# helloybz/CLANE

Measured on AMD Instinct MI355X. Metric: embedding-update iters/sec (Jacobi sweeps of Z <- X + gamma*P*Z, P frozen), higher is better.
Workload: dtype f32; 1 GPU; R-MAT |V|=2000000 |E|=40000000 d=256 f32, gamma=0.76, CosineSimilarity (reference mode), seeds 3/4

## Files before the change

### clane_amd/_hip.py

```python
from __future__ import annotations

import abc
import ctypes as C
import os
import threading
from pathlib import Path
from typing import Optional

import torch

LIB_NAME = "libclane_hip.so"
LIB_PATH = Path(__file__).resolve().parent / LIB_NAME
ABI_VERSION = 5

SCORE_REFERENCE, SCORE_PER_EDGE, SCORE_RAW_DOT = 0, 1, 2
SPMM_SINKS_UNTOUCHED = 1
SPMM_TABLE_BEYOND_CACHE = 2
SCORE_FUSE_SOFTMAX = 1
SCORE_MODES = {"reference": SCORE_REFERENCE, "per_edge": SCORE_PER_EDGE, "raw_dot": SCORE_RAW_DOT}

_p, _i64, _i32 = C.c_void_p, C.c_int64, C.c_int32

SIGNATURES = {
    "clane_abi_version": (C.c_int, []),
# ... 29 lines not shown
    SIGNATURES[f"clane_spmm_update_class_{_s}"] = (
        C.c_int,
        [_p, _p, _p, _p, _p, _i64, _i32, _p, _p, _i64, _i64, _p, _i64, _p, _i64, _g, _p, _i64, _i32, _i32, _p, _p, _p, _p])
    SIGNATURES[f"clane_edge_score_class_{_s}"] = (
        C.c_int, [_p, _p, _p, _p, _p, _p, _i64, _i32, _p, _p, _i64, _i64, _p, _i64, _i32, _i32, _p, _p, _p, _i32, _p, _p])
    SIGNATURES[f"clane_gather_rows_{_s}"] = (C.c_int, [_p, _i64, _p, _i64, _i32, _p, _i64, _p])
    SIGNATURES[f"clane_l1_distance_{_s}"] = (C.c_int, [_p, _i64, _p, _i64, _i64, _i32, _p, _p, _p, _p])
for _s in ("f32", "f64"):
    SIGNATURES[f"clane_degree_weighted_sums_{_s}"] = (C.c_int, [_p, _p, _p, _i64, _p, _p, _p])
    SIGNATURES[f"clane_edge_score_finalize_{_s}"] = (C.c_int, [_p, _p, _i64, _i64, _i32, _p, _p, _p, _p])
    SIGNATURES[f"clane_segment_softmax_{_s}"] = (C.c_int, [_p, _i64, _p, _i64, _i64, _p, _i64, _p])
    SIGNATURES[f"clane_pair_cosine_{_s}"] = (C.c_int, [_p, _i64, _p, _i64, _i64, _i32, _p, _p, _p])
    SIGNATURES[f"clane_edge_score_pair_{_s}"] = (
        C.c_int, [_p, _p, _i64, _i64, _p, _i64, _p, _i64, _i32, _p, _i32, _i64, _p, _i64, _p])
    SIGNATURES[f"clane_edge_score_class_pair_{_s}"] = (
        C.c_int, [_p, _p, _p, _p, _p, _p, _i64, _i32, _p, _p, _i64, _i64, _p, _i64, _p, _i64, _i32, _p, _i32, _p, _p])
for _s in ("f32", "f64", "bf16"):
    SIGNATURES[f"clane_project_rows_{_s}"] = (C.c_int, [_p, _i64, _i32, _i64, _p, _p, _i64, _p])
    SIGNATURES[f"clane_pair_project_{_s}"] = (C.c_int, [_p, _i64, _i32, _i64, _p, _p, _i64, _p, _p, _p, _p])
    SIGNATURES[f"clane_pair_grad_{_s}"] = (C.c_int, [_p, _i64, _i32, _i64, _p, _p, _i64, _p, _p, _p, _p, _p, _p, _p])
for _s in ("f32", "f64"):
    SIGNATURES[f"clane_pair_loss_{_s}"] = (C.c_int, [_p, _p, _i64, _i32, _p, _p, _p, _p, _p, _p, _p])
    SIGNATURES[f"clane_adam_step_{_s}"] = (C.c_int, [_p, _p, _p, _p, _i64, C.c_double, _p, _p, _p])
SIGNATURES["clane_pair_grad_ws_len"] = (_i64, [_i64, _i32])
SIGNATURES["clane_pair_labels"] = (C.c_int, [_p, _p, _i64, _p, _p, _i64, _p, _p])

_SUFFIX = {torch.float32: "f32", torch.float64: "f64", torch.bfloat16: "bf16"}
_ACC = {torch.float32: torch.float32, torch.float64: torch.float64, torch.bfloat16: torch.float32}
VEC_ELEMS = {torch.float32: 4, torch.float64: 2, torch.bfloat16: 8}


class ClaneHipError(RuntimeError):
    pass


class _MirrorStruct(C.Structure):
    _fields_ = [("row_ptr", _p), ("slot", _p), ("bufs", _p), ("ld", _i64), ("aligned16", _i32)]


MIRROR_ROW_BITS = 28


class Mirror:

    def __init__(self, row_ptr: torch.Tensor, slot: torch.Tensor, bufs):
        if row_ptr.dtype != torch.int64 or slot.dtype != torch.int32 or not (row_ptr.is_contiguous()
# ... 204 lines not shown
    def edge_score_class_pair(self, rowptr, colidx, item_e0, item_len, item_slot, item_row, items_per_block,
                              class_rows, slot_ptr, row0, S, N, d, scores, stats=None, fuse_softmax=False,
                              n_slots=None, row_parts=1):
        raise NotImplementedError(f"{type(self).__name__} has no edge_score_class_pair")

    def pair_project(self, Z, d: int, src, dst, W, A, Bm):
        raise NotImplementedError(f"{type(self).__name__} has no pair_project")

    def pair_loss(self, A, Bm, d: int, linked, u, g, mask, ws, stats):
        raise NotImplementedError(f"{type(self).__name__} has no pair_loss")

    def pair_grad_ws_len(self, B: int, d: int) -> int:
        raise NotImplementedError(f"{type(self).__name__} has no pair_grad_ws_len")

    def pair_grad(self, Z, d: int, src, dst, A, Bm, g, stats, ws, dW):
        raise NotImplementedError(f"{type(self).__name__} has no pair_grad")

    def adam_step(self, W, m, v, dW, lr: float, stats, state):
        raise NotImplementedError(f"{type(self).__name__} has no adam_step")

    def pair_labels(self, rowptr, colidx, nrows: int, src, dst, linked):
        raise NotImplementedError(f"{type(self).__name__} has no pair_labels")

    def bind(self, method: str, *args, **kwargs):
        fn = getattr(self, method)
        return lambda: fn(*args, **kwargs)


class HipKernels(KernelBackend):

    def __init__(self, lib: Optional[C.CDLL] = None):
        self.lib = lib if lib is not None else load_library()
        self._tls = threading.local()

    def _invoke(self, fn, what: str, *cargs):
        rec = getattr(self._tls, "recording", None)
        if rec is not None:
            rec.append((fn, cargs, what))
        else:
            self._check(fn(*cargs), what)

    def bind(self, method: str, *args, **kwargs):
        self._tls.recording = []
        try:
            getattr(self, method)(*args, **kwargs)
            (fn, cargs, what), = self._tls.recording
        finally:
            self._tls.recording = None
        check = self._check
        return lambda: check(fn(*cargs), what)

    def _check(self, rc: int, what: str):
# ... 136 lines not shown
                     _mirror_arg(mirror, Z_new.dtype), _vec(partials, torch.float64, "partials"), self._stream(Z_old))

    def spmm_split_slab_len(self, n_segments: int, d: int) -> int:
        return int(self.lib.clane_spmm_split_slab_len(n_segments, d))

    def spmm_update_split(self, rowptr, colidx, P, split_rows, seg_ptr, seg_row, edges_per_segment: int, row0: int,
                          Z_old, X, gamma: float, Z_new, d: int, slab, partials, mirror: Optional[Mirror] = None):
        zo, ldz = _mat(Z_old, "Z_old")
        xp, ldx = _mat(X, "X")
        zn, ldo = _mat(Z_new, "Z_new")
        self._invoke(self._fn("clane_spmm_update_split", Z_old.dtype), "clane_spmm_update_split",
                     _vec(rowptr, torch.int64, "rowptr"), _vec(colidx, torch.int32, "colidx"),
                     _vec(P, acc_dtype(Z_old.dtype), "P"), _vec(split_rows, torch.int32, "split_rows"),
                     _vec(seg_ptr, torch.int64, "seg_ptr"), _vec(seg_row, torch.int32, "seg_row"),
                     split_rows.numel(), seg_row.numel(), edges_per_segment, row0, zo, ldz, xp, ldx, gamma, zn, ldo, d,
                     _vec(slab, acc_dtype(Z_old.dtype), "slab"), _mirror_arg(mirror, Z_new.dtype),
                     _vec(partials, torch.float64, "partials"), self._stream(Z_old))

    def spmm_class_slab_len(self, n_slots: int, d: int) -> int:
        return int(self.lib.clane_spmm_class_slab_len(n_slots, d))

    def spmm_update_class(self, colidx, P, item_e0, item_len, item_slot, items_per_block: int, class_rows, slot_ptr,
                          row0: int, Z_old, X, gamma: float, Z_new, d: int, slab, partials,
                          mirror: Optional[Mirror] = None, beyond_cache: bool = False):
        zo, ldz = _mat(Z_old, "Z_old")
        xp, ldx = _mat(X, "X")
        zn, ldo = _mat(Z_new, "Z_new")
        n_items = item_e0.numel()
        if n_items % items_per_block or item_len.numel() != n_items or item_slot.numel() != n_items:
            raise ValueError("spmm_update_class: the item arrays must hold whole blocks of items_per_block items")
        self._invoke(self._fn("clane_spmm_update_class", Z_old.dtype), "clane_spmm_update_class",
                     _vec(colidx, torch.int32, "colidx"), _vec(P, acc_dtype(Z_old.dtype), "P"),
                     _vec(item_e0, torch.int64, "item_e0"), _vec(item_len, torch.int32, "item_len"),
                     _vec(item_slot, torch.int32, "item_slot"), n_items // items_per_block, items_per_block,
                     _vec(class_rows, torch.int32, "class_rows"), _vec(slot_ptr, torch.int64, "slot_ptr"),
                     class_rows.numel(), row0, zo, ldz, xp, ldx, gamma, zn, ldo, d,
                     SPMM_TABLE_BEYOND_CACHE if beyond_cache else 0,
                     _vec(slab, acc_dtype(Z_old.dtype), "slab"), _mirror_arg(mirror, Z_new.dtype),
                     _vec(partials, torch.float64, "partials"), self._stream(Z_old))

    def reduce_partials(self, partials, n: int, ws, out):
        self._invoke(self.lib.clane_reduce_partials, "clane_reduce_partials",
                     _vec(partials, torch.float64, "partials"), n, _vec(ws, torch.float64, "ws"),
                     _vec(out, torch.float64, "out"), self._stream(out))

    def l1_distance(self, A, B, d: int, ws, out, sq_a: Optional[torch.Tensor] = None):
        ap, lda = _mat(A, "A")
        bp, ldb = _mat(B, "B")
        self._check(self._fn("clane_l1_distance", A.dtype)(
            ap, lda, bp, ldb, A.shape[0], d, self._sq_arg(sq_a, A.dtype), _vec(ws, torch.float64, "ws"),
            _vec(out, torch.float64, "out"), self._stream(A)), "clane_l1_distance")

    def gather_rows(self, src, idx, d: int, dst):
# ... 144 lines not shown
```

### clane_amd/csrc/clane_abi.hip

```cpp
#include "../../include/clane_hip.h"

#include <hip/hip_runtime.h>

#include <climits>
#include <cstdarg>
#include <cstdio>
#include <cstring>

#include "build_p.h"
#include "edge_score.h"
#include "device_utils.h"
#include "pair_train.h"
#include "projection.h"
#include "spmm_update.h"

namespace {

using namespace clane;

thread_local char g_err[512] = "";

int fail(int code, const char *fmt, ...) {
    va_list ap;
    va_start(ap, fmt);
// ... 446 lines not shown
    const Layout L = pick_layout<T>(d, {Z_old, X, Z_new, mirror_alignment_probe(mirror, Z_new)},
                                    {ldz, ldx, ldo, mirror && mirror->row_ptr ? mirror->ld : ldo});
    const int64_t ld_slab = ceil_div(d, 8) * 8;
    const Mirror<T> mir = make_mirror<T>(mirror);
    dispatch_layout<T>(L, [&]<int VEC, int LPR>() {
        constexpr int U = VEC > 1 ? CLANE_LONG_U : 4;
        constexpr int kDeepU = (LPR == 32 && VEC == 4 && sizeof(T) == 4) ? CLANE_CLASS_U32
                               : (LPR == 16 && VEC == 8 && sizeof(T) == 2) ? CLANE_CLASS_U16B : 0;
        if (n_blocks > 0 && kDeepU > 0 && (flags & CLANE_SPMM_TABLE_BEYOND_CACHE))
            spmm_class_chunk_kernel<T, PT, VEC, LPR, (kDeepU > 0 ? kDeepU : U)>
                <<<unsigned(n_blocks), kBlock, 0, (hipStream_t)stream>>>(
                    colidx, P, item_e0, item_len, item_slot, items_per_block, Z_old, ldz, d, slab, ld_slab);
        else if (n_blocks > 0)
            spmm_class_chunk_kernel<T, PT, VEC, LPR, U><<<unsigned(n_blocks), kBlock, 0, (hipStream_t)stream>>>(
                colidx, P, item_e0, item_len, item_slot, items_per_block, Z_old, ldz, d, slab, ld_slab);
        spmm_class_combine_kernel<T, VEC, LPR>
            <<<unsigned(ceil_div(n_rows, kWave / LPR)), kCombineWaves * kWave, 0, (hipStream_t)stream>>>(
            class_rows, slot_ptr, n_rows, row0, slab, ld_slab, Z_old, ldz, X, ldx, gamma, Z_new, ldo, d, mir,
            (flags & CLANE_SPMM_TABLE_BEYOND_CACHE) != 0, delta_partials);
    });
    return check_launch("spmm_update_class");
}

template <typename T>
int l1_distance(const T *A, int64_t lda, const T *B, int64_t ldb, int64_t nrows, int32_t d,
                typename Elem<T>::acc_t *sq_a, double *ws, double *out, void *stream) {
    REQUIRE(nrows >= 0 && d > 0 && lda >= d && ldb >= d, "l1_distance: bad shape");
    REQUIRE(ws && out, "l1_distance: null workspace/output");
    REQUIRE(nrows == 0 || (A && B), "l1_distance: null pointer");
    const Layout L = pick_layout<T>(d, {A, B}, {lda, ldb});
    if (sq_a != nullptr) {
        const Layout LA = pick_layout<T>(d, {A}, {lda});
        REQUIRE(LA.vec == L.vec && LA.lpr == L.lpr,
                "l1_distance: sq_a needs B as aligned as A (the lane layout of row_sqnorm on A)");
    }
    int grid = 1;
    dispatch_layout<T>(L, [&]<int VEC, int LPR>() {
        grid = grid_for_waves(ceil_div(nrows > 0 ? nrows : 1, (kWave / LPR) * stream_rows(LPR)));
        if (grid > kReduceGrid) grid = kReduceGrid;
        l1_distance_kernel<T, VEC, LPR><<<grid, kBlock, 0, (hipStream_t)stream>>>(A, lda, B, ldb, nrows, d, sq_a, ws);
    });
    reduce_fixed_kernel<<<1, 1024, 0, (hipStream_t)stream>>>(ws, grid, grid, 1, out);
    return check_launch("l1_distance");
}

template <typename T>
// ... 302 lines not shown
CLANE_SPLIT_WRAPPER(f32, float, float, float, float)
CLANE_SPLIT_WRAPPER(f64, double, double, double, double)
CLANE_SPLIT_WRAPPER(bf16, uint16_t, bf16_t, float, float)
#undef CLANE_SPLIT_WRAPPER
#define CLANE_CLASS_WRAPPER(SUF, CT, T, PT, GT)                                                                        \
    int clane_spmm_update_class_##SUF(const int32_t *colidx, const PT *P, const int64_t *item_e0,                     \
                                      const int32_t *item_len, const int32_t *item_slot, int64_t n_blocks,            \
                                      int32_t items_per_block, const int32_t *class_rows, const int64_t *slot_ptr,    \
                                      int64_t n_rows, int64_t row0, const CT *Z_old, int64_t ldz, const CT *X,        \
                                      int64_t ldx, GT gamma, CT *Z_new, int64_t ldo, int32_t d, int32_t flags,        \
                                      GT *slab, const clane_mirror_t *mirror, double *delta_partials, void *stream) { \
        return spmm_update_class<T, PT>(colidx, P, item_e0, item_len, item_slot, n_blocks, items_per_block,           \
                                        class_rows, slot_ptr, n_rows, row0, reinterpret_cast<const T *>(Z_old), ldz,  \
                                        reinterpret_cast<const T *>(X), ldx, gamma, reinterpret_cast<T *>(Z_new),     \
                                        ldo, d, flags, slab, mirror, delta_partials, stream);                         \
    }
CLANE_CLASS_WRAPPER(f32, float, float, float, float)
CLANE_CLASS_WRAPPER(f64, double, double, double, double)
CLANE_CLASS_WRAPPER(bf16, uint16_t, bf16_t, float, float)
#undef CLANE_CLASS_WRAPPER
int64_t clane_spmm_class_slab_len(int64_t n_slots, int32_t d) { return n_slots * (ceil_div(d, 8) * 8); }
int64_t clane_spmm_split_slab_len(int64_t n_segments, int32_t d) { return n_segments * (ceil_div(d, 8) * 8); }

CLANE_SPMM_WRAPPERS(f32, float, float, float, float)
CLANE_SPMM_WRAPPERS(f64, double, double, double, double)
CLANE_SPMM_WRAPPERS(bf16, uint16_t, bf16_t, float, float)
#undef CLANE_SPMM_WRAPPERS

int clane_reduce_partials(const double *partials, int64_t n, double *ws, double *out, void *stream) {
    if (n < 0 || !out || !ws || (n > 0 && !partials))
        return fail(CLANE_ERR_INVALID_ARGUMENT, "reduce_partials: bad arguments");
    if (n <= 8192) {
        reduce_fixed_kernel<<<1, 1024, 0, (hipStream_t)stream>>>(partials, n, n, 1, out);
    } else {
        const int64_t slice = ceil_div(n, kReduceGrid);
        const int grid = int(ceil_div(n, slice));
        reduce_slices_kernel<<<grid, kBlock, 0, (hipStream_t)stream>>>(partials, n, slice, ws);
        reduce_fixed_kernel<<<1, 1024, 0, (hipStream_t)stream>>>(ws, grid, grid, 1, out);
    }
    return check_launch("reduce_partials");
}

int clane_l1_distance_f32(const float *A, int64_t lda, const float *B, int64_t ldb, int64_t nrows, int32_t d,
                          float *sq_a, double *ws, double *out, void *stream) {
    return l1_distance<float>(A, lda, B, ldb, nrows, d, sq_a, ws, out, stream);
}
// ... 74 lines not shown
```

### clane_amd/csrc/spmm_update.h

```cpp
#pragma once

#include "device_utils.h"

#ifndef CLANE_SPMM_U
#define CLANE_SPMM_U 8
#endif
#ifndef CLANE_SPMM_DYNAMIC
#define CLANE_SPMM_DYNAMIC 1
#endif
#ifndef CLANE_COMBINE_WAVES
#define CLANE_COMBINE_WAVES 2
#endif
#ifndef CLANE_SPMM_PREFETCH
#define CLANE_SPMM_PREFETCH 1
#endif
#ifndef CLANE_SPMM_MIN_WAVES
#define CLANE_SPMM_MIN_WAVES 0
#endif

namespace clane {

template <typename A>
struct EdgeChunk {
    int c;
// ... 624 lines not shown
            for (int t0 = 0; t0 < d; t0 += LPR * VEC) {
                const int c0 = t0 + sl * VEC;
                const bool col_ok = c0 < d;
                A acc[VEC];
#pragma unroll
                for (int k = 0; k < VEC; ++k) acc[k] = A(0);
                gather_accumulate<T, PT, VEC, LPR, U>(colidx, P, e0, e1, Zold + (col_ok ? c0 : 0), ldz, col_ok, acc, ch, true);
                fold_subwaves<LPR>(acc);
                if (col_ok && sub == 0) {
                    Pack<A, VEC> o;
#pragma unroll
                    for (int k = 0; k < VEC; ++k) o.v[k] = acc[k];
                    slab_store<A, VEC>(out + c0, o);
                }
            }
        }
        cur = nxt;
        e0 = n0;
        e1 = n1;
        ch = chn;
    }
}

constexpr int kCombineWaves = CLANE_COMBINE_WAVES;
#ifndef CLANE_COMBINE_LOADS
#define CLANE_COMBINE_LOADS 16
#endif
constexpr int kCombineLoads = CLANE_COMBINE_LOADS;

template <typename T, int VEC, int LPR>
__global__ __launch_bounds__(kCombineWaves *kWave) void spmm_class_combine_kernel(
    const int32_t *__restrict__ class_rows, const int64_t *__restrict__ slot_ptr, int64_t n_rows, int64_t row0,
    const typename Elem<T>::acc_t *__restrict__ slab, int64_t ld_slab, const T *__restrict__ Zold, int64_t ldz,
    const T *__restrict__ X, int64_t ldx, typename Elem<T>::acc_t gamma, T *__restrict__ Znew, int64_t ldo, int d,
    Mirror<T> mirror, bool nt_store, double *__restrict__ partials) {
    using A = typename Elem<T>::acc_t;
    constexpr int kRows = kWave / LPR;
    __shared__ A s_part[kCombineWaves > 1 ? kCombineWaves - 1 : 1][kWave][VEC];
    const int lane = lane_id();
    const int wave = __builtin_amdgcn_readfirstlane(threadIdx.x / kWave);
    const int sub = lane / LPR, sl = lane % LPR;
    const int64_t i = int64_t(blockIdx.x) * kRows + sub;
    const bool live = i < n_rows;
    const int64_t r = live ? class_rows[i] : 0;
    const int64_t s0 = live ? slot_ptr[i] : 0, s1 = live ? slot_ptr[i + 1] : 0;
    const int64_t share = ceil_div(s1 - s0, int64_t(kCombineWaves));
// ... 62 lines not shown
```

### clane_amd/diagnostics.py

```python
from __future__ import annotations

import numpy as np

from .plan import lanes_per_row


class DiagnosticsMixin:

    def kernel_times_ms(self):
        t = np.array([(e0.elapsed_time(e4), e4.elapsed_time(e1), e1.elapsed_time(e2), e2.elapsed_time(e3))
                      for _, e0, e1, e2, e3, e4 in self.kernel_events]).reshape(-1, 4)
        self.kernel_events = []
        if not len(t):
            return {}
        per_sweep = t.reshape(-1, len(self.blocks), 4).sum(1).mean(0)
        return dict(zip(("split", "hub", "mid", "main"), per_sweep.tolist()))

    def collective_times_ms(self):
        ev, self.collective_events = self.collective_events, []
        if not ev:
            return {}
        t = np.array([(a.elapsed_time(b), b.elapsed_time(c)) for a, b, c in ev])
        return {"exchange_exposed": float(t[:, 0].mean()), "allreduce": float(t[:, 1].mean()), "sweeps_timed": len(ev)}

# ... 19 lines not shown
                "mid": "spmm_long_kernel<4 waves>", "hub": "spmm_long_kernel<16 waves>",
                "split": "spmm_class_chunk_kernel+combine" if self.class_threshold > 0
                else "spmm_split_segment_kernel+combine"}

    def estimated_sweep_seconds(self) -> float:
        s = self.Zcur.element_size()
        d = self.d_full
        total = self.E_total * (d * s + 8) + self.V * 3 * d * s
        return total / max(self.world, 1) / 8e12

    def kernel_config(self) -> dict:
        return {"build": self.k.build_info(), "dtype": str(self.dtype).replace("torch.", ""), "d": self.d,
                "lanes_per_row": lanes_per_row(self.d, self.dtype) if self.d > 0 else 0,
                "rows": int(self.part.n_local), "edges": int(self.E_loc), "launch_blocks": len(self.blocks),
                "long_threshold": self.long_threshold, "score_threshold": self.score_threshold,
                "hub_threshold": self.hub_threshold,
                "split_edges": self.split_edges, "segment_edges": self.segment_edges,
                "class_threshold": self.class_threshold, "class_chunk": self.class_chunk, "class_k1": self.class_k1,
                "class_phases": self.class_phases, "phase_threshold": self.phase_threshold,
                "class_of_row": "xor-fold of 3-bit groups" if self.class_threshold else None,
                "class_affinity": self.class_affinity, "mega_segment_edges": self.mega_segment_edges,
                "class_items_per_block": [c[6] for c in self.class_rows if c is not None][:1],
                "column_tiles": len(self.tiles),
                "fewer_loads_in_flight": bool(self.beyond_cache and self.d > 0 and (str(self.dtype), lanes_per_row(
                    self.d_plan if len(self.tiles) > 1 else self.d, self.dtype)) in (("torch.float32", 32), ("torch.bfloat16", 16))),
                "hot_rows_first": self.hot_rows_first, "exchange": self.exchange,
                }

    def exchange_bytes_per_sweep(self) -> int:
        s = self.Zcur.element_size()
        if self.halo:
            return self.part.recv_rows_per_sweep() * self.ld * s
        if self.columns:
            return 0
        return sum((b.span[1] - b.span[0] - b.nrows) * self.ld * s for b in self.blocks if b.span is not None)
```

### clane_amd/engine.py

```python
from __future__ import annotations

import contextlib
import threading
from typing import List, Optional

import numpy as np
import torch

from . import _hip, xcd
from .comm import TorchComm
from .diagnostics import DiagnosticsMixin
from .halo import build_halo_layout
from .partition import Block, HostCSR, LocalCSR, RowPartition, localize
from .plan import (HEAVY_ROW_EDGES, HUB_FACTOR, INFINITY_CACHE_BYTES, L2_BYTES_ALL_XCDS,
                   LONG_THRESHOLD_BY_ROWS_PER_WAVE, MIN_HOT_READ_SHARE, MIN_SEGMENT_EDGES, MIN_SLICE_ROW_BYTES,
                   SOFTMAX_EDGES_PER_WORKGROUP, SPLIT_EDGES, TARGET_SEGMENTS, UNSKEWED_LONG_THRESHOLD, _round_up,
                   column_slice, hot_read_share, lanes_per_row, pick_exchange)
from .staging import StagedZ, StagingMixin, place_piece
from .xcd import (CLASS_CHUNK, CLASS_THRESHOLD_BY_ROWS_PER_WAVE, PHASE_THRESHOLD, PHASES_BY_ROWS_PER_WAVE,
                  class_items)

class SweepEngine(StagingMixin, DiagnosticsMixin):
    STAGE_SLOTS = 3
    N_TABLES = 3
    MAX_TIMED_SWEEPS = 32

    EXCHANGES = ("auto", "columns", "halo", "halo_p2p", "allgather", "allgather_all")

    def __init__(self, csr: HostCSR, X: torch.Tensor, device, kernels=None, *, cosine_mode: str = "reference",
                 process_group=None, chunks: Optional[int] = None, long_threshold: Optional[int] = None,
                 hub_threshold: Optional[int] = None, shuffle: Optional[bool] = None, seed: int = 0,
                 exchange: str = "auto", comm=None, hot_rows_first: bool = True, split_hubs: bool = True,
                 overlap_chunks: bool = True, fused_pack: bool = True, class_threshold: Optional[int] = None,
                 class_chunk: int = CLASS_CHUNK, class_k1: bool = True, class_phases: Optional[int] = None,
                 phase_threshold: int = PHASE_THRESHOLD, delta_stream: bool = False, table_skew=None,
                 table_alloc: str = "torch", column_tiles: Optional[int] = None):
        if X.dim() != 2 or X.shape[0] != csr.num_vertices:
            raise ValueError(f"X must be [V, d] with V={csr.num_vertices}, got {tuple(X.shape)}")
        if cosine_mode not in ("reference", "per_edge"):
            raise ValueError(f"cosine_mode must be 'reference' or 'per_edge', got {cosine_mode!r}")
        csr.validate()
        csr.indeg(device)
        self.k = kernels if kernels is not None else _hip.kernels()
        self.device = torch.device(device)
        self.dtype = X.dtype
        self.acc_dtype = _hip.acc_dtype(X.dtype)
        self.cosine_mode = cosine_mode
        self.table_skew = table_skew
        if table_alloc not in ("torch", "contiguous"):
            raise ValueError("table_alloc must be 'torch' or 'contiguous'")
        self.table_alloc, self._own_tables, self.table_alloc_note = table_alloc, [], None
        self._column_tiles_asked = column_tiles
        X = self._choose_division(csr, X, process_group, comm, exchange)
        self._choose_class_pass(csr, class_threshold, class_chunk, class_k1, class_phases, phase_threshold)
        self._build_layout(csr, chunks, shuffle, seed, hot_rows_first)
        self._choose_row_bins(long_threshold, hub_threshold)
        deg = self._upload_structure()
        self._bin_rows(deg, split_hubs)
        self._setup_exchange(deg, fused_pack)
        self._alloc_tables(X, deg)
        self._alloc_scratch(delta_stream, overlap_chunks)
        self._Y = None

    def _choose_division(self, csr: HostCSR, X: torch.Tensor, process_group, comm, exchange: str) -> torch.Tensor:
        self.pg = process_group
        self.comm = comm if comm is not None else (TorchComm(process_group) if process_group is not None else None)
        self.world = self.comm.world if self.comm is not None else 1
        rank = self.comm.rank if self.comm is not None else 0
        if exchange not in self.EXCHANGES:
            raise ValueError("exchange must be 'auto', 'columns', 'halo', 'halo_p2p', 'allgather' or "
                             f"'allgather_all', got {exchange!r}")
        self._forced = self.world == 1 and self.comm is not None and bool(self.comm.force) and exchange in (
            "columns", "allgather", "allgather_all")
        divided = self.world > 1 or self._forced
        if exchange == "auto":
            exchange = pick_exchange(int(X.shape[1]), X.dtype, self.world)
        self._exchange_asked = exchange
        self.exchange = exchange if divided else "none"
        self.columns = divided and exchange == "columns"
        self.C = self.world if self.columns else 1
        self.c = rank if self.columns else 0
        self.V, self.d_full = csr.num_vertices, int(X.shape[1])
# ... 42 lines not shown
        self.class_affinity = True
        if class_threshold is None:
            class_threshold = CLASS_THRESHOLD_BY_ROWS_PER_WAVE[self.rows_per_wave]
            if self.rows_per_wave == 2 and csr.num_vertices * row_bytes <= INFINITY_CACHE_BYTES:
                class_threshold = max(class_threshold, 128)
            if self.hot_read_share < MIN_HOT_READ_SHARE:
                class_threshold = max(class_threshold, HEAVY_ROW_EDGES)
                self.class_affinity = False
        self.class_threshold = int(class_threshold)
        self.class_chunk = int(class_chunk)
        self.class_k1 = bool(class_k1) and self.class_threshold > 0
        if class_phases is None:
            class_phases = (xcd.PHASES_UNDER_COLUMN_TILES if len(self.tiles) > 1 else 0) or \
                PHASES_BY_ROWS_PER_WAVE[self.rows_per_wave]
        self.class_phases = int(class_phases)
        if self.class_threshold == 0 or self.class_phases < 1:
            self.class_phases = 1
        if self.class_phases & (self.class_phases - 1) or self.class_phases > 8:
            raise ValueError("class_phases must be 1, 2, 4 or 8")
        self.phase_threshold = max(int(phase_threshold), self.class_threshold) if self.class_phases > 1 else 0
        if self.class_threshold and not (64 <= self.class_chunk <= 4096 and self.class_chunk % 64 == 0):
            raise ValueError("class_chunk must be a multiple of 64 in [64, 4096]")
        self.mega_segment_edges = int(L2_BYTES_ALL_XCDS // 8 // max(row_bytes, 1)) if self.d_plan > 0 else 0

    def _build_layout(self, csr: HostCSR, chunks, shuffle, seed: int, hot_rows_first: bool) -> None:
        if chunks is None:
            chunks = 1 if self.row_world == 1 else 4
        self.hot_rows_first = bool(hot_rows_first)
        if self.halo:
            self.part = build_halo_layout(csr, self.row_world, self.row_rank, chunks, shuffle=shuffle is not False, seed=seed,
                                          hot_rows_first=hot_rows_first, class_threshold=self.class_threshold,
                                          phase_threshold=self.phase_threshold, phases=self.class_phases)
            self.blocks: List[Block] = self.part.blocks
            self.local: LocalCSR = self.part.local
        else:
            live = csr.live_mask() if (self.row_world > 1 and self._exchange_asked == "allgather") else None
            hot = csr.indeg() if (self.row_world == 1 and hot_rows_first and not shuffle) else None
            self.part = RowPartition.create(self.V, self.row_world, self.row_rank, chunks, live_mask=live, shuffle=shuffle,
                                            seed=seed, priority=hot)
            self.blocks = self.part.blocks(spans_for_one_rank=self._forced and not self.columns)
            self.local = localize(csr, self.part, self.device, class_threshold=self.class_threshold,
                                  phase_threshold=self.phase_threshold, phases=self.class_phases)
        if self.part.padded_vertices >= 2 ** 31:
            raise ValueError(f"{self.part.padded_vertices} table rows: column indices are 32-bit (ABI v1); divide the "
                             "rows over more GPUs (exchange='halo') or wait for 64-bit indices")

# ... 396 lines not shown
                rp, Xb, Zn = self.rowptr[b.local_start:], self.X_loc[self._rows(b)], self._zrows(Znew, b)
                po = self.partial_off[i]
                mir = self.mirrors_p2p[dst][i] if self.p2p else self.mirrors[i]
                po_mid = po + k.spmm_partials_len(b.nrows, 0)
                po_hub = po_mid + (0 if self.mid_rows[i] is None else self.mid_rows[i].numel())
                po_split = po_hub + (0 if self.hub_rows[i] is None else self.hub_rows[i].numel())
                po_class = po_split + (0 if self.split_rows[i] is None else self.split_rows[i][0].numel())
                steps.append(("event", i, 0))
                if self.d == 0:
                    per_block.append(steps + [("event", i, e) for e in (4, 1, 2, 3)])
                    continue
                T = len(self.tiles)
                cut = (lambda M, t: M) if T == 1 else (lambda M, t: M[:, self.tiles[t][0]:self.tiles[t][1]])
                width = (lambda t: self.d) if T == 1 else (lambda t: self.tiles[t][1] - self.tiles[t][0])
                part = lambda off, t: self.partials[t * self.partial_off[-1] + off:]
                if mir is not None and T > 1:
                    raise AssertionError("column tiles and mirrored launches do not combine")
                for t in range(T):
                    if self.class_rows[i] is not None:
                        rows_c, slot_ptr, it_e0, it_len, it_slot, _, ipb = self.class_rows[i]
                        steps.append(("call", self._bind("spmm_update_class", self.colidx, self.P, it_e0, it_len, it_slot,
                                                         ipb, rows_c, slot_ptr, b.row0, cut(Zold, t), cut(Xb, t), gamma,
                                                         cut(Zn, t), width(t), self.slabs[i % len(self.slabs)],
                                                         part(po_class, t), mirror=mir, beyond_cache=self.beyond_cache)))
                    if self.split_rows[i] is not None:
                        rows_s, seg_ptr, seg_row = self.split_rows[i]
                        steps.append(("call", self._bind("spmm_update_split", rp, self.colidx, self.P, rows_s, seg_ptr,
                                                         seg_row, self.segment_edges, b.row0, cut(Zold, t), cut(Xb, t), gamma,
                                                         cut(Zn, t), width(t), self.slabs[i % len(self.slabs)],
                                                         part(po_split, t), mirror=mir)))
                steps.append(("event", i, 4))
                for t in range(T):
                    if self.hub_rows[i] is not None:
                        steps.append(("call", self._bind("spmm_update_long", rp, self.colidx, self.P, self.hub_rows[i], 16,
                                                         b.row0, cut(Zold, t), cut(Xb, t), gamma, cut(Zn, t), width(t),
                                                         part(po_hub, t), mirror=mir)))
                steps.append(("event", i, 1))
                for t in range(T):
                    if self.mid_rows[i] is not None:
                        steps.append(("call", self._bind("spmm_update_long", rp, self.colidx, self.P, self.mid_rows[i], 4,
                                                         b.row0, cut(Zold, t), cut(Xb, t), gamma, cut(Zn, t), width(t),
                                                         part(po_mid, t), mirror=mir)))
                steps.append(("event", i, 2))
                for t in range(T):
                    steps.append(("call", self._bind("spmm_update", rp, self.colidx, self.P, b.nrows, b.row0, cut(Zold, t),
                                                     cut(Xb, t), gamma, cut(Zn, t), width(t), self.long_threshold,
                                                     part(po, t), sinks_untouched=True, mirror=mir,
                                                     beyond_cache=self.beyond_cache)))
                steps.append(("event", i, 3))
                if b.span is not None:
                    steps.append(("allgather", Znew[b.span[0]:b.span[1]], Zn))
                elif b.exchange is not None and not self.p2p:
                    ex = b.exchange
                    if self.send_rows[i] is not None and mir is None:
                        steps.append(("call", self._bind("gather_rows", Znew, self.send_rows[i], self.d,
                                                         self.send_buf[i])))
                    steps.append(("alltoall", Znew[ex.recv_start:ex.recv_start + ex.recv_rows], self.send_buf[i],
                                  ex.out_splits, ex.in_splits))
            per_block.append(steps)
        final = self._bind("reduce_partials", self.partials, self.partials.numel(), self.ws,
                           self.delta_pp[tick:tick + 1])
        return per_block, final

    def sweep(self, gamma: float) -> float:
        return self.sweep_wait(self.sweep_launch(gamma))

    def sweep_launch(self, gamma: float) -> int:
        if not self.P_valid:
            raise RuntimeError("sweep() before build_P()")
        stream = torch.cuda.current_stream(self.device).cuda_stream if self.device.type == "cuda" else 0
        src = self.cur
        dst = next(i for i in range(len(self.Zbuf)) if i != src and i != self.hold)
        parity = self._tick
        self._tick ^= 1
        if self._delta_stream is not None and self._delta_busy[parity]:
            torch.cuda.current_stream(self.device).wait_event(self._delta_ev[parity])
            self._delta_busy[parity] = False
        key = (src, dst, parity, float(gamma), stream)
        plan = self._plans.get(key)
        if plan is None:
            plan = self._plans[key] = self._build_plan(src, dst, parity, float(gamma))
        events = None
        if self.time_kernels and len(self.kernel_events) < self.MAX_TIMED_SWEEPS * len(self.blocks):
            events = [[torch.cuda.Event(enable_timing=True) for _ in range(5)] for _ in self.blocks]
            self.kernel_events.extend((i,) + tuple(ev) for i, ev in enumerate(events))
# ... 101 lines not shown
```

### clane_amd/xcd.py

```python
from __future__ import annotations

from typing import Optional

import numpy as np
import torch

XCD_CLASSES = 8


def xcd_class(position):
    p = position
    return (p ^ (p >> 3) ^ (p >> 6) ^ (p >> 9)) & (XCD_CLASSES - 1)


def xcd_subclass(position, row_degree, class_threshold: int, phase_threshold: int = 0, phases: int = 1):
    cls = xcd_class(position)
    if phases > 1 and phase_threshold > 0:
        cls = cls + XCD_CLASSES * (((position >> 6) % phases) * (row_degree > phase_threshold))
    return cls * (row_degree > class_threshold)


CLASS_THRESHOLD_BY_ROWS_PER_WAVE = {1: 64, 2: 64, 4: 256, 8: 256}
CLASS_CHUNK = 256
PHASES_BY_ROWS_PER_WAVE = {1: 4, 2: 2, 4: 1, 8: 1}
PHASES_UNDER_COLUMN_TILES = 0
PHASE_THRESHOLD = 512
CLASS_ITEMS_PIECE_EDGES = 1 << 28
CLASS_ITEMS_PER_BLOCK = 16



def row_pieces(rowptr: np.ndarray, max_edges: int):
    n = rowptr.size - 1
    a = 0
    while a < n:
        b = int(np.searchsorted(rowptr, rowptr[a] + max_edges, side="right")) - 1
        b = min(max(b, a + 1), n)
        yield a, b
        a = b


def class_items(rowptr: np.ndarray, colidx: np.ndarray, rows: np.ndarray, chunk: int, items_per_block: Optional[int],
                row_ids: Optional[np.ndarray] = None, colidx_dev: Optional[torch.Tensor] = None,
                phase_threshold: int = 0, phases: int = 1, mega_segment_edges: int = 0, mega_min_edges: int = 0) -> dict:
    n = rows.size
    NS = XCD_CLASSES * max(1, phases)
    sizes = (rowptr[rows + 1] - rowptr[rows]).astype(np.int64)
    start = np.concatenate([[0], np.cumsum(sizes)[:-1]])
    if colidx_dev is not None and colidx_dev.is_cuda:
        dev = colidx_dev.device
        seg_len = np.empty(n * NS, dtype=np.int64)
        unsorted = False
# ... 75 lines not shown
```

### include/clane_hip.h

```cpp
#ifndef CLANE_HIP_H_
#define CLANE_HIP_H_

#include <stdint.h>

#ifdef __cplusplus
extern "C" {
#endif

#define CLANE_ABI_VERSION 5

#define CLANE_OK 0
#define CLANE_ERR_INVALID_ARGUMENT (-1)
#define CLANE_ERR_LAUNCH (-2)

#define CLANE_SCORE_REFERENCE 0
#define CLANE_SCORE_PER_EDGE 1
#define CLANE_SCORE_RAW_DOT 2

#define CLANE_SCORE_FUSE_SOFTMAX 1
#define CLANE_SCORE_ROW_PARTS(n) (((n) & 0xff) << 8)

#define CLANE_SPMM_SINKS_UNTOUCHED 1
#define CLANE_SPMM_TABLE_BEYOND_CACHE 2

// ... 116 lines not shown
                                const int64_t *slot_ptr, int64_t n_rows, int64_t row0, const uint16_t *Z, int64_t ldz,
                                int32_t d, int32_t mode, const double *sums2, const float *sq, float *scores,
                                int32_t flags, float *stats, void *stream);

int64_t clane_spmm_class_slab_len(int64_t n_slots, int32_t d);
int clane_spmm_update_class_f32(const int32_t *colidx, const float *P, const int64_t *item_e0, const int32_t *item_len,
                                const int32_t *item_slot, int64_t n_blocks, int32_t items_per_block,
                                const int32_t *class_rows, const int64_t *slot_ptr, int64_t n_rows, int64_t row0,
                                const float *Z_old, int64_t ldz, const float *X, int64_t ldx, float gamma, float *Z_new,
                                int64_t ldo, int32_t d, int32_t flags, float *slab, const clane_mirror_t *mirror,
                                double *delta_partials, void *stream);
int clane_spmm_update_class_f64(const int32_t *colidx, const double *P, const int64_t *item_e0, const int32_t *item_len,
                                const int32_t *item_slot, int64_t n_blocks, int32_t items_per_block,
                                const int32_t *class_rows, const int64_t *slot_ptr, int64_t n_rows, int64_t row0,
                                const double *Z_old, int64_t ldz, const double *X, int64_t ldx, double gamma,
                                double *Z_new, int64_t ldo, int32_t d, int32_t flags, double *slab, const clane_mirror_t *mirror,
                                double *delta_partials, void *stream);
int clane_spmm_update_class_bf16(const int32_t *colidx, const float *P, const int64_t *item_e0, const int32_t *item_len,
                                 const int32_t *item_slot, int64_t n_blocks, int32_t items_per_block,
                                 const int32_t *class_rows, const int64_t *slot_ptr, int64_t n_rows, int64_t row0,
                                 const uint16_t *Z_old, int64_t ldz, const uint16_t *X, int64_t ldx, float gamma,
                                 uint16_t *Z_new, int64_t ldo, int32_t d, int32_t flags, float *slab, const clane_mirror_t *mirror,
                                 double *delta_partials, void *stream);

int clane_reduce_partials(const double *partials, int64_t n, double *ws, double *out, void *stream);

int clane_l1_distance_f32(const float *A, int64_t lda, const float *B, int64_t ldb, int64_t nrows, int32_t d,
                          float *sq_a, double *ws, double *out, void *stream);
int clane_l1_distance_f64(const double *A, int64_t lda, const double *B, int64_t ldb, int64_t nrows, int32_t d,
                          double *sq_a, double *ws, double *out, void *stream);
int clane_l1_distance_bf16(const uint16_t *A, int64_t lda, const uint16_t *B, int64_t ldb, int64_t nrows, int32_t d,
                           float *sq_a, double *ws, double *out, void *stream);

int clane_gather_rows_f32(const float *src, int64_t lds, const int32_t *idx, int64_t n, int32_t d, float *dst,
                          int64_t ldd, void *stream);
int clane_gather_rows_f64(const double *src, int64_t lds, const int32_t *idx, int64_t n, int32_t d, double *dst,
                          int64_t ldd, void *stream);
int clane_gather_rows_bf16(const uint16_t *src, int64_t lds, const int32_t *idx, int64_t n, int32_t d, uint16_t *dst,
                           int64_t ldd, void *stream);

int clane_pair_cosine_f32(const float *A, int64_t lda, const float *B, int64_t ldb, int64_t nrows, int32_t d,
                          float *out, double *ws, void *stream);
int clane_pair_cosine_f64(const double *A, int64_t lda, const double *B, int64_t ldb, int64_t nrows, int32_t d,
                          double *out, double *ws, void *stream);

int clane_project_rows_f32(const float *Z, int64_t rows, int32_t d, int64_t ldz, const float *W, float *Y, int64_t ldy,
// ... 58 lines not shown
```

Before: 274.1 sweeps/s.

## Serve hottest per-class neighbour rows from LDS in the class SpMM pass

Adds a new fp32 class-pass kernel that preloads each XCD class's top hot rows of Z_old (up to 2048 rows across the 8 classes, 256 per class) into LDS. Column indices of those hot rows are encoded as negative values so the gather reads them from shared memory instead of L2/HBM. The kernel also runs as a persistent grid that claims work items through an LDS atomic counter, with the next item's edge chunk prefetched. It is enabled by default when the engine uses class affinity with hot-rows-first ordering. The trade-off is a per-workgroup LDS fill and much lower occupancy from the large LDS allocation, plus an extra select per gathered element.

```diff
diff --git a/clane_amd/_hip.py b/clane_amd/_hip.py
--- a/clane_amd/_hip.py
+++ b/clane_amd/_hip.py
@@ -75,6 +75,9 @@
 for _s in ("f32", "f64"):
     SIGNATURES[f"clane_pair_loss_{_s}"] = (C.c_int, [_p, _p, _i64, _i32, _p, _p, _p, _p, _p, _p, _p])
     SIGNATURES[f"clane_adam_step_{_s}"] = (C.c_int, [_p, _p, _p, _p, _i64, C.c_double, _p, _p, _p])
+SIGNATURES["clane_spmm_update_class_lds_f32"] = (
+    C.c_int, [_p, _p, _p, _p, _p, _i64, _i32, _p, _p, _i64, _i64, _p, _i64, _p, _i64, C.c_float, _p, _i64, _i32, _i32, _i32,
+              _i32, _i32, _p, _p, _p, _p])
 SIGNATURES["clane_pair_grad_ws_len"] = (_i64, [_i64, _i32])
 SIGNATURES["clane_pair_labels"] = (C.c_int, [_p, _p, _i64, _p, _p, _i64, _p, _p])
 
@@ -325,12 +328,16 @@
     def pair_labels(self, rowptr, colidx, nrows: int, src, dst, linked):
         raise NotImplementedError(f"{type(self).__name__} has no pair_labels")
 
+    class_lds = False
+
     def bind(self, method: str, *args, **kwargs):
         fn = getattr(self, method)
         return lambda: fn(*args, **kwargs)
 
 
 class HipKernels(KernelBackend):
+
+    class_lds = True
 
     def __init__(self, lib: Optional[C.CDLL] = None):
         self.lib = lib if lib is not None else load_library()
@@ -513,13 +520,29 @@
 
     def spmm_update_class(self, colidx, P, item_e0, item_len, item_slot, items_per_block: int, class_rows, slot_ptr,
                           row0: int, Z_old, X, gamma: float, Z_new, d: int, slab, partials,
-                          mirror: Optional[Mirror] = None, beyond_cache: bool = False):
+                          mirror: Optional[Mirror] = None, beyond_cache: bool = False, hot_rows: int = 0,
+                          workgroups: int = 0, waves: int = 0):
         zo, ldz = _mat(Z_old, "Z_old")
         xp, ldx = _mat(X, "X")
         zn, ldo = _mat(Z_new, "Z_new")
         n_items = item_e0.numel()
         if n_items % items_per_block or item_len.numel() != n_items or item_slot.numel() != n_items:
             raise ValueError("spmm_update_class: the item arrays must hold whole blocks of items_per_block items")
+        if hot_rows > 0:
+            if Z_old.dtype != torch.float32:
+                raise ValueError("spmm_update_class: hot_rows needs float32 tables")
+            if hot_rows > Z_old.shape[0]:
+                raise ValueError("spmm_update_class: hot_rows exceeds the table's rows")
+            self._invoke(self.lib.clane_spmm_update_class_lds_f32, "clane_spmm_update_class_lds_f32",
+                         _vec(colidx, torch.int32, "colidx"), _vec(P, torch.float32, "P"),
+                         _vec(item_e0, torch.int64, "item_e0"), _vec(item_len, torch.int32, "item_len"),
+                         _vec(item_slot, torch.int32, "item_slot"), n_items // items_per_block, items_per_block,
+                         _vec(class_rows, torch.int32, "class_rows"), _vec(slot_ptr, torch.int64, "slot_ptr"),
+                         class_rows.numel(), row0, zo, ldz, xp, ldx, gamma, zn, ldo, d,
+                         SPMM_TABLE_BEYOND_CACHE if beyond_cache else 0, hot_rows, workgroups, waves,
+                         _vec(slab, torch.float32, "slab"), _mirror_arg(mirror, Z_new.dtype),
+                         _vec(partials, torch.float64, "partials"), self._stream(Z_old))
+            return
         self._invoke(self._fn("clane_spmm_update_class", Z_old.dtype), "clane_spmm_update_class",
                      _vec(colidx, torch.int32, "colidx"), _vec(P, acc_dtype(Z_old.dtype), "P"),
                      _vec(item_e0, torch.int64, "item_e0"), _vec(item_len, torch.int32, "item_len"),
diff --git a/clane_amd/csrc/clane_abi.hip b/clane_amd/csrc/clane_abi.hip
--- a/clane_amd/csrc/clane_abi.hip
+++ b/clane_amd/csrc/clane_abi.hip
@@ -492,6 +492,77 @@
     return check_launch("spmm_update_class");
 }
 
+constexpr int kLdsBytesPerCu = 160 * 1024;
+inline bool class_lds_layout(const Layout &L) { return L.vec && L.lpr == 32; }
+
+template <int WAVES>
+int launch_class_chunk_lds(const int32_t *colidx, const float *P, const int64_t *item_e0, const int32_t *item_len,
+                           const int32_t *item_slot, int64_t n_blocks, int32_t items_per_block, const float *Z_old,
+                           int64_t ldz, int32_t d, int32_t flags, float *slab, int64_t ld_slab, int32_t hot_rows,
+                           int32_t workgroups, void *stream) {
+    constexpr int VEC = 4, LPR = 32;
+    constexpr int U = (CLANE_CLASS_U32 > 0) ? CLANE_CLASS_U32 : CLANE_LONG_U;
+    const size_t lds = size_t(hot_rows / 8) * LPR * 16;
+    auto go = [&](auto kernel) -> int {
+        static bool raised = false;
+        if (!raised) {
+            const hipError_t e = hipFuncSetAttribute(reinterpret_cast<const void *>(kernel),
+                                                     hipFuncAttributeMaxDynamicSharedMemorySize, kLdsBytesPerCu - 1024);
+            if (e != hipSuccess) return fail(CLANE_ERR_LAUNCH, "spmm_update_class_lds: %s", hipGetErrorString(e));
+            raised = true;
+        }
+        kernel<<<unsigned(workgroups), WAVES * kWave, lds, (hipStream_t)stream>>>(
+            colidx, P, item_e0, item_len, item_slot, items_per_block, int(n_blocks / 8), Z_old, ldz, d, slab, ld_slab,
+            hot_rows);
+        return CLANE_OK;
+    };
+    if (flags & CLANE_SPMM_TABLE_BEYOND_CACHE) return go(spmm_class_chunk_lds_kernel<float, float, VEC, LPR, U, WAVES>);
+    return go(spmm_class_chunk_lds_kernel<float, float, VEC, LPR, CLANE_LONG_U, WAVES>);
+}
+
+int spmm_update_class_lds(const int32_t *colidx, const float *P, const int64_t *item_e0, const int32_t *item_len,
+                          const int32_t *item_slot, int64_t n_blocks, int32_t items_per_block, const int32_t *class_rows,
+                          const int64_t *slot_ptr, int64_t n_rows, int64_t row0, const float *Z_old, int64_t ldz,
+                          const float *X, int64_t ldx, float gamma, float *Z_new, int64_t ldo, int32_t d, int32_t flags,
+                          int32_t hot_rows, int32_t workgroups, int32_t waves, float *slab, const clane_mirror_t *mirror,
+                          double *delta_partials, void *stream) {
+    REQUIRE(hot_rows >= 0 && hot_rows % 8 == 0, "spmm_update_class_lds: hot_rows must be a multiple of 8");
+    const Layout L = d > 0 ? pick_layout<float>(d, {Z_old, X, Z_new, mirror_alignment_probe(mirror, Z_new)},
+                                                {ldz, ldx, ldo, mirror && mirror->row_ptr ? mirror->ld : ldo})
+                           : Layout{false, 64};
+    if (hot_rows == 0 || n_blocks <= 0 || n_rows <= 0 || !class_lds_layout(L))
+        return spmm_update_class<float, float>(colidx, P, item_e0, item_len, item_slot, n_blocks, items_per_block,
+                                               class_rows, slot_ptr, n_rows, row0, Z_old, ldz, X, ldx, gamma, Z_new, ldo,
+                                               d, flags, slab, mirror, delta_partials, stream);
+    REQUIRE(mirror_ok(mirror, d), "spmm_update_class_lds: incomplete mirror descriptor");
+    REQUIRE(n_blocks <= INT32_MAX && n_blocks % 8 == 0 && n_rows <= INT32_MAX && row0 >= 0,
+            "spmm_update_class_lds: bad shape (n_blocks must be a multiple of 8)");
+    REQUIRE(items_per_block >= kWavesPerBlock && items_per_block <= kMaxItemsPerBlock,
+            "spmm_update_class_lds: items_per_block must be in [%d, %d]", kWavesPerBlock, kMaxItemsPerBlock);
+    REQUIRE(ldz >= d && ldx >= d && ldo >= d, "spmm_update_class_lds: leading dimension < d");
+    REQUIRE(colidx && P && item_e0 && item_len && item_slot && class_rows && slot_ptr && Z_old && X && Z_new && slab &&
+                delta_partials,
+            "spmm_update_class_lds: null pointer");
+    REQUIRE((const void *)Z_new != (const void *)Z_old, "spmm_update_class_lds: Z_new must not alias Z_old");
+    REQUIRE(aligned16(slab), "spmm_update_class_lds: slab must be 16-byte aligned");
+    REQUIRE(workgroups >= 8 && workgroups % 8 == 0 && workgroups <= kMaxGrid,
+            "spmm_update_class_lds: workgroups must be a multiple of 8 in [8, %d]", kMaxGrid);
+    REQUIRE(waves == 8 || waves == 16, "spmm_update_class_lds: waves must be 8 or 16");
+    REQUIRE(int64_t(hot_rows / 8) * 32 * 16 <= kLdsBytesPerCu - 1024,
+            "spmm_update_class_lds: %d hot rows do not fit one CU's LDS", hot_rows);
+    const int64_t ld_slab = ceil_div(d, 8) * 8;
+    const int rc = waves == 16 ? launch_class_chunk_lds<16>(colidx, P, item_e0, item_len, item_slot, n_blocks, items_per_block,
+                                                            Z_old, ldz, d, flags, slab, ld_slab, hot_rows, workgroups, stream)
+                               : launch_class_chunk_lds<8>(colidx, P, item_e0, item_len, item_slot, n_blocks, items_per_block,
+                                                           Z_old, ldz, d, flags, slab, ld_slab, hot_rows, workgroups, stream);
+    if (rc != CLANE_OK) return rc;
+    spmm_class_combine_kernel<float, 4, 32>
+        <<<unsigned(ceil_div(n_rows, kWave / 32)), kCombineWaves * kWave, 0, (hipStream_t)stream>>>(
+            class_rows, slot_ptr, n_rows, row0, slab, ld_slab, Z_old, ldz, X, ldx, gamma, Z_new, ldo, d,
+            make_mirror<float>(mirror), (flags & CLANE_SPMM_TABLE_BEYOND_CACHE) != 0, delta_partials);
+    return check_launch("spmm_update_class_lds");
+}
+
 template <typename T>
 int l1_distance(const T *A, int64_t lda, const T *B, int64_t ldb, int64_t nrows, int32_t d,
                 typename Elem<T>::acc_t *sq_a, double *ws, double *out, void *stream) {
@@ -840,6 +911,18 @@
 int64_t clane_spmm_class_slab_len(int64_t n_slots, int32_t d) { return n_slots * (ceil_div(d, 8) * 8); }
 int64_t clane_spmm_split_slab_len(int64_t n_segments, int32_t d) { return n_segments * (ceil_div(d, 8) * 8); }
 
+int clane_spmm_update_class_lds_f32(const int32_t *colidx, const float *P, const int64_t *item_e0, const int32_t *item_len,
+                                    const int32_t *item_slot, int64_t n_blocks, int32_t items_per_block,
+                                    const int32_t *class_rows, const int64_t *slot_ptr, int64_t n_rows, int64_t row0,
+                                    const float *Z_old, int64_t ldz, const float *X, int64_t ldx, float gamma,
+                                    float *Z_new, int64_t ldo, int32_t d, int32_t flags, int32_t hot_rows,
+                                    int32_t workgroups, int32_t waves, float *slab, const clane_mirror_t *mirror,
+                                    double *delta_partials, void *stream) {
+    return spmm_update_class_lds(colidx, P, item_e0, item_len, item_slot, n_blocks, items_per_block, class_rows, slot_ptr,
+                                 n_rows, row0, Z_old, ldz, X, ldx, gamma, Z_new, ldo, d, flags, hot_rows, workgroups, waves,
+                                 slab, mirror, delta_partials, stream);
+}
+
 CLANE_SPMM_WRAPPERS(f32, float, float, float, float)
 CLANE_SPMM_WRAPPERS(f64, double, double, double, double)
 CLANE_SPMM_WRAPPERS(bf16, uint16_t, bf16_t, float, float)
diff --git a/clane_amd/csrc/spmm_update.h b/clane_amd/csrc/spmm_update.h
--- a/clane_amd/csrc/spmm_update.h
+++ b/clane_amd/csrc/spmm_update.h
@@ -670,6 +670,135 @@
     }
 }
 
+
+__device__ __forceinline__ int class_row_position(int r, int cls) {
+    return (r << 3) | (cls ^ ((r ^ (r >> 3) ^ (r >> 6)) & 7));
+}
+__device__ __forceinline__ int class_of_position(int p) { return (p ^ (p >> 3) ^ (p >> 6) ^ (p >> 9)) & 7; }
+
+template <typename T, int VEC, int LPR, int U>
+__device__ __forceinline__ void accumulate_chunk_hot(const EdgeChunk<typename Elem<T>::acc_t> &ch, int n,
+                                                     const T *__restrict__ zcol, int64_t ldz, bool col_ok,
+                                                     const T *hot, typename Elem<T>::acc_t (&acc)[VEC]) {
+    using A = typename Elem<T>::acc_t;
+    constexpr int EPW = kWave / LPR;
+    const int sub = lane_id() / LPR;
+    for (int j = 0; j < n; j += EPW * U) {
+        Pack<T, VEC> z[U], zh[U];
+        A pj[U];
+        int cj[U];
+        bool live[U];
+#pragma unroll
+        for (int u = 0; u < U; ++u) {
+            const int idx = j + u * EPW + sub;
+            cj[u] = lane_get(ch.c, idx & (kWave - 1));
+            const A pv = lane_get(ch.p, idx & (kWave - 1));
+            live[u] = idx < n && col_ok;
+            pj[u] = idx < n ? pv : A(0);
+        }
+#pragma unroll
+        for (int u = 0; u < U; ++u) {
+            z[u] = Pack<T, VEC>{};
+            if (live[u] && cj[u] >= 0) z[u] = load_pack<T, VEC>(zcol + int64_t(cj[u]) * ldz);
+        }
+#pragma unroll
+        for (int u = 0; u < U; ++u) zh[u] = load_pack<T, VEC>(hot + (cj[u] < 0 ? ~cj[u] : 0) * (LPR * VEC));
+#pragma unroll
+        for (int u = 0; u < U; ++u) {
+            const bool from_lds = live[u] && cj[u] < 0;
+#pragma unroll
+            for (int k = 0; k < VEC; ++k)
+                acc[k] = fma(pj[u], Elem<T>::to_acc(from_lds ? zh[u].v[k] : z[u].v[k]), acc[k]);
+        }
+    }
+}
+
+template <typename T, typename PT, int VEC, int LPR, int U, int WAVES>
+__global__ __launch_bounds__(WAVES *kWave) void spmm_class_chunk_lds_kernel(
+    const int32_t *__restrict__ colidx, const PT *__restrict__ P, const int64_t *__restrict__ item_e0,
+    const int32_t *__restrict__ item_len, const int32_t *__restrict__ item_slot, int items_per_block,
+    int blocks_per_class, const T *__restrict__ Zold, int64_t ldz, int d, typename Elem<T>::acc_t *__restrict__ slab,
+    int64_t ld_slab, int hot_rows) {
+    using A = typename Elem<T>::acc_t;
+    static_assert(LPR < kWave && VEC == Elem<T>::kVec, "16-byte packs, rows of at most half a wave");
+    extern __shared__ __align__(16) unsigned char s_raw[];
+    __shared__ int s_next;
+    T *const s_hot = reinterpret_cast<T *>(s_raw);
+    const int lane = lane_id();
+    const int wave = __builtin_amdgcn_readfirstlane(threadIdx.x / kWave);
+    const int sub = lane / LPR;
+    const int sl = lane % LPR;
+    const int c0 = sl * VEC;
+    const bool col_ok = c0 < d;
+    const int cls = blockIdx.x % 8, j0 = blockIdx.x / 8, stride = gridDim.x / 8;
+
+    const int n_packs = (hot_rows >> 3) * LPR;
+#pragma unroll 4
+    for (int i = threadIdx.x; i < n_packs; i += WAVES * kWave) {
+        const int r = i / LPR, l = i % LPR;
+        Pack<T, VEC> v{};
+        if (l * VEC < d) v = load_pack<T, VEC>(Zold + int64_t(class_row_position(r, cls)) * ldz + l * VEC);
+        store_pack<T, VEC>(s_hot + int64_t(i) * VEC, v);
+    }
+    if (threadIdx.x == 0) s_next = WAVES;
+    __syncthreads();
+
+    const int my_blocks = j0 < blocks_per_class ? (blocks_per_class - j0 + stride - 1) / stride : 0;
+    const int total = my_blocks * items_per_block;
+    struct Item {
+        int64_t e0;
+        int len, slot;
+    };
+    auto describe = [&](int v) -> Item {
+        if (v >= total) return Item{0, 0, -1};
+        const int64_t i = (int64_t(j0 + (v / items_per_block) * stride) * 8 + cls) * items_per_block + v % items_per_block;
+        return Item{item_e0[i], item_len[i], item_slot[i]};
+    };
+    auto claim = [&]() -> int {
+        int v = 0;
+        if (lane == 0) v = atomicAdd(&s_next, 1);
+        return __builtin_amdgcn_readfirstlane(v);
+    };
+    auto encode = [&](int c) -> int { return (c < hot_rows && class_of_position(c) == cls) ? ~(c >> 3) : c; };
+
+    int cur = wave;
+    Item it = describe(cur);
+    EdgeChunk<A> ch = load_chunk<A, PT>(colidx, P, it.e0, it.e0 + it.len);
+    int nxt = cur < total ? claim() : total;
+    Item itn = describe(nxt);
+    while (cur < total) {
+        const int nn = nxt < total ? claim() : total;
+        const Item itnn = describe(nn);
+        const EdgeChunk<A> chn = load_chunk<A, PT>(colidx, P, itn.e0, itn.e0 + itn.len);
+        if (it.len > 0) {
+            const int64_t e0 = it.e0, e1 = it.e0 + it.len;
+            A acc[VEC];
+#pragma unroll
+            for (int k = 0; k < VEC; ++k) acc[k] = A(0);
+            for (int64_t e = e0; e < e1; e += kWave) {
+                const int64_t left = e1 - e;
+                const int n = left < kWave ? int(left) : kWave;
+                EdgeChunk<A> c = ch;
+                if (e != e0) c = load_chunk<A, PT>(colidx, P, e, e1);
+                c.c = encode(c.c);
+                accumulate_chunk_hot<T, VEC, LPR, U>(c, n, Zold + (col_ok ? c0 : 0), ldz, col_ok, s_hot + c0, acc);
+            }
+            fold_subwaves<LPR>(acc);
+            if (col_ok && sub == 0) {
+                Pack<A, VEC> o;
+#pragma unroll
+                for (int k = 0; k < VEC; ++k) o.v[k] = acc[k];
+                slab_store<A, VEC>(slab + int64_t(it.slot) * ld_slab + c0, o);
+            }
+        }
+        cur = nxt;
+        it = itn;
+        ch = chn;
+        nxt = nn;
+        itn = itnn;
+    }
+}
+
 constexpr int kCombineWaves = CLANE_COMBINE_WAVES;
 #ifndef CLANE_COMBINE_LOADS
 #define CLANE_COMBINE_LOADS 16
diff --git a/clane_amd/diagnostics.py b/clane_amd/diagnostics.py
--- a/clane_amd/diagnostics.py
+++ b/clane_amd/diagnostics.py
@@ -65,6 +65,8 @@
                 "class_affinity": self.class_affinity, "mega_segment_edges": self.mega_segment_edges,
                 "class_items_per_block": [c[6] for c in self.class_rows if c is not None][:1],
                 "column_tiles": len(self.tiles),
+                **({"class_hot_rows": self.class_hot_rows,
+                    "class_lds_grid": [self.class_lds_workgroups, self.class_lds_waves]} if self.class_hot_rows else {}),
                 "fewer_loads_in_flight": bool(self.beyond_cache and self.d > 0 and (str(self.dtype), lanes_per_row(
                     self.d_plan if len(self.tiles) > 1 else self.d, self.dtype)) in (("torch.float32", 32), ("torch.bfloat16", 16))),
                 "hot_rows_first": self.hot_rows_first, "exchange": self.exchange,
diff --git a/clane_amd/engine.py b/clane_amd/engine.py
--- a/clane_amd/engine.py
+++ b/clane_amd/engine.py
@@ -34,7 +34,7 @@
                  overlap_chunks: bool = True, fused_pack: bool = True, class_threshold: Optional[int] = None,
                  class_chunk: int = CLASS_CHUNK, class_k1: bool = True, class_phases: Optional[int] = None,
                  phase_threshold: int = PHASE_THRESHOLD, delta_stream: bool = False, table_skew=None,
-                 table_alloc: str = "torch", column_tiles: Optional[int] = None):
+                 table_alloc: str = "torch", column_tiles: Optional[int] = None, class_hot_rows: Optional[int] = None):
         if X.dim() != 2 or X.shape[0] != csr.num_vertices:
             raise ValueError(f"X must be [V, d] with V={csr.num_vertices}, got {tuple(X.shape)}")
         if cosine_mode not in ("reference", "per_edge"):
@@ -58,6 +58,7 @@
         deg = self._upload_structure()
         self._bin_rows(deg, split_hubs)
         self._setup_exchange(deg, fused_pack)
+        self._choose_class_lds(class_hot_rows, shuffle)
         self._alloc_tables(X, deg)
         self._alloc_scratch(delta_stream, overlap_chunks)
         self._Y = None
@@ -146,6 +147,25 @@
         if self.class_threshold and not (64 <= self.class_chunk <= 4096 and self.class_chunk % 64 == 0):
             raise ValueError("class_chunk must be a multiple of 64 in [64, 4096]")
         self.mega_segment_edges = int(L2_BYTES_ALL_XCDS // 8 // max(row_bytes, 1)) if self.d_plan > 0 else 0
+
+    def _choose_class_lds(self, class_hot_rows: Optional[int], shuffle) -> None:
+        width = self.d_plan if len(self.tiles) > 1 else self.d
+        able = (self.k.class_lds and self.device.type == "cuda" and self.class_threshold > 0
+                and self.dtype == torch.float32 and width > 0 and lanes_per_row(width, self.dtype) == 32
+                and self.world == 1 and not self._forced and all(m is None for m in self.mirrors))
+        if class_hot_rows is None:
+            wanted = xcd.CLASS_LDS_HOT_ROWS if (able and self.class_affinity and self.hot_rows_first and not shuffle) else 0
+        else:
+            wanted = int(class_hot_rows)
+            if wanted < 0 or wanted % 8:
+                raise ValueError("class_hot_rows must be a non-negative multiple of 8")
+            if wanted and not able:
+                raise ValueError("class_hot_rows: this engine's class pass cannot serve rows from LDS (fp32 rows of "
+                                 "257..512 bytes per tile on one GPU with the native kernels only)")
+        self.class_hot_rows = min(wanted, xcd.CLASS_LDS_MAX_HOT_ROWS, self.part.padded_vertices // 8 * 8)
+        big = self.class_hot_rows > xcd.CLASS_LDS_MAX_HOT_ROWS // 2
+        self.class_lds_waves = 16 if big else 8
+        self.class_lds_workgroups = xcd.CLASS_LDS_CUS * (1 if big else 2)
 
     def _build_layout(self, csr: HostCSR, chunks, shuffle, seed: int, hot_rows_first: bool) -> None:
         if chunks is None:
@@ -588,7 +608,8 @@
                         steps.append(("call", self._bind("spmm_update_class", self.colidx, self.P, it_e0, it_len, it_slot,
                                                          ipb, rows_c, slot_ptr, b.row0, cut(Zold, t), cut(Xb, t), gamma,
                                                          cut(Zn, t), width(t), self.slabs[i % len(self.slabs)],
-                                                         part(po_class, t), mirror=mir, beyond_cache=self.beyond_cache)))
+                                                         part(po_class, t), mirror=mir, beyond_cache=self.beyond_cache,
+                                                         **self._class_lds_args())))
                     if self.split_rows[i] is not None:
                         rows_s, seg_ptr, seg_row = self.split_rows[i]
                         steps.append(("call", self._bind("spmm_update_split", rp, self.colidx, self.P, rows_s, seg_ptr,
@@ -627,6 +648,11 @@
         final = self._bind("reduce_partials", self.partials, self.partials.numel(), self.ws,
                            self.delta_pp[tick:tick + 1])
         return per_block, final
+
+    def _class_lds_args(self) -> dict:
+        if not self.class_hot_rows:
+            return {}
+        return dict(hot_rows=self.class_hot_rows, workgroups=self.class_lds_workgroups, waves=self.class_lds_waves)
 
     def sweep(self, gamma: float) -> float:
         return self.sweep_wait(self.sweep_launch(gamma))
diff --git a/clane_amd/xcd.py b/clane_amd/xcd.py
--- a/clane_amd/xcd.py
+++ b/clane_amd/xcd.py
@@ -28,6 +28,17 @@
 CLASS_ITEMS_PIECE_EDGES = 1 << 28
 CLASS_ITEMS_PER_BLOCK = 16
 
+CLASS_LDS_HOT_ROWS = 2048
+CLASS_LDS_MAX_HOT_ROWS = 2048
+CLASS_LDS_CUS = 256
+
+
+def class_rank(position):
+    return xcd_class(position), position >> 3
+
+
+def class_row_position(rank, cls):
+    return (rank << 3) | (cls ^ ((rank ^ (rank >> 3) ^ (rank >> 6)) & (XCD_CLASSES - 1)))
 
 
 def row_pieces(rowptr: np.ndarray, max_edges: int):
diff --git a/include/clane_hip.h b/include/clane_hip.h
--- a/include/clane_hip.h
+++ b/include/clane_hip.h
@@ -162,6 +162,14 @@
                                  const uint16_t *Z_old, int64_t ldz, const uint16_t *X, int64_t ldx, float gamma,
                                  uint16_t *Z_new, int64_t ldo, int32_t d, int32_t flags, float *slab, const clane_mirror_t *mirror,
                                  double *delta_partials, void *stream);
+
+int clane_spmm_update_class_lds_f32(const int32_t *colidx, const float *P, const int64_t *item_e0, const int32_t *item_len,
+                                    const int32_t *item_slot, int64_t n_blocks, int32_t items_per_block,
+                                    const int32_t *class_rows, const int64_t *slot_ptr, int64_t n_rows, int64_t row0,
+                                    const float *Z_old, int64_t ldz, const float *X, int64_t ldx, float gamma,
+                                    float *Z_new, int64_t ldo, int32_t d, int32_t flags, int32_t hot_rows,
+                                    int32_t workgroups, int32_t waves, float *slab, const clane_mirror_t *mirror,
+                                    double *delta_partials, void *stream);
 
 int clane_reduce_partials(const double *partials, int64_t n, double *ws, double *out, void *stream);
 
```

After: 257.2 sweeps/s. -6.2%, worse.
